# Pi-Star-Lab/RESCO

Hardware: AMD Instinct MI355X
Metric: env-steps/sec (higher is better)
Workload: dtype f32; 1 GPU; ingolstadt21 x 4096 lock-step envs per GPU (BASELINE config 3), fixed demand from the map's rou.xml, on-device seeded random policy, Krauss sigma 0.5 + speedFactor dev 0.1; tls_expiry=1, map=ingolstadt21, envs_per_gpu=4096, pipes=2, ticks_per_env_step=10, block_threads=512, lds_bytes_per_env=40896, parallelism=env-batch split x1, no collective on the data path

## Files before the change

resco_amd/csrc/resco_sim.hip:

```cpp
#include <hip/hip_runtime.h>
#include <hip/hip_fp16.h>
#include <stdint.h>
#include <stdio.h>
#include <stdlib.h>
#include <string.h>
#include <mutex>
#include <new>
#include <string>
#include <vector>

#include "resco_sim.h"

#define RS_DEV __device__ __forceinline__
#define RS_HD __host__ __device__
#define RS_MEM __device__ __forceinline__
#define RS_G(p) (p)
#define RS_CARVE __host__ __device__ __forceinline__
__device__ __forceinline__ void rs_atomic_min(int32_t *p, int32_t v) { atomicMin(p, v); }
__device__ __forceinline__ void rs_atomic_min(uint32_t *p, uint32_t v) { atomicMin(p, v); }
__device__ __forceinline__ void rs_atomic_max(int32_t *p, int32_t v) { atomicMax(p, v); }
__device__ __forceinline__ void rs_atomic_add(int32_t *p, int32_t v) { atomicAdd(p, v); }
__device__ __forceinline__ int32_t rs_atomic_fetch_add(int32_t *p, int32_t v) { return atomicAdd(p, v); }
__device__ __forceinline__ int32_t rs_wave_ticket(int32_t *p) {
    const unsigned long long m = __ballot(1);
    const int below = (int)__builtin_amdgcn_mbcnt_hi((uint32_t)(m >> 32), __builtin_amdgcn_mbcnt_lo((uint32_t)m, 0u));
    int32_t base = 0;
    if (below == 0) base = atomicAdd(p, (int32_t)__popcll(m));
    return __builtin_amdgcn_readlane(base, __ffsll((long long)m) - 1) + below;
}
__device__ __forceinline__ void rs_wave_add(int32_t *p, int32_t v) {
    for (int m = 32; m > 0; m >>= 1) v += __shfl_xor(v, m);
    if ((threadIdx.x & 63) == 0 && v) atomicAdd(p, v);
}
__device__ __forceinline__ void rs_wave_max(int32_t *p, int32_t v) {
    for (int m = 32; m > 0; m >>= 1) { const int32_t o = __shfl_xor(v, m); v = o > v ? o : v; }
    if ((threadIdx.x & 63) == 0) atomicMax(p, v);
}
__device__ __forceinline__ void rs_atomic_or(uint32_t *p, uint32_t v) { atomicOr(p, v); }
__device__ __forceinline__ uint32_t rs_atomic_fetch_or(uint32_t *p, uint32_t v) { return atomicOr(p, v); }
__device__ __forceinline__ int rs_atomic_inc(int32_t *p) { return atomicAdd(p, 1); }
__device__ __forceinline__ void rs_atomic_and(uint32_t *p, uint32_t v) { atomicAnd(p, v); }
__device__ __forceinline__ uint32_t rs_atomic_cas(uint32_t *p, uint32_t cmp, uint32_t v) { return atomicCAS(p, cmp, v); }
__device__ __forceinline__ int rs_ffsll(unsigned long long x) { return __ffsll(x); }
__device__ __forceinline__ int rs_clzll(unsigned long long x) { return __clzll((long long)x); }
__device__ __forceinline__ int rs_ffs(uint32_t x) { return __ffs((int)x); }
__device__ __forceinline__ int rs_popc(uint32_t x) { return __popc(x); }
__device__ __forceinline__ float rs_int_as_float(int x) { return __int_as_float(x); }
__device__ __forceinline__ int rs_float_as_int(float x) { return __float_as_int(x); }
__device__ __forceinline__ uint16_t rs_f2h(float x) { return __half_as_ushort(__float2half(x)); }

#ifndef RS_IEEE_DIV
__device__ __forceinline__ float rs_div_unscaled(float a, float b) {
    const float r0 = __builtin_amdgcn_rcpf(b);
    const float r1 = __builtin_fmaf(__builtin_fmaf(-b, r0, 1.0f), r0, r0);
    const float q0 = a * r1;
    const float q1 = __builtin_fmaf(__builtin_fmaf(-b, q0, a), r1, q0);
    return __builtin_fmaf(__builtin_fmaf(-b, q1, a), r1, q1);
}
#define RS_DIV(a, b) rs_div_unscaled((a), (b))
#endif
#define RS_OPAQUE_S(x) asm volatile("" : "+s"(x));
#ifndef RS_NARROW_NODE
#define RS_KEEP4(a, b, c, d) asm volatile("" : "+v"(a), "+v"(b), "+v"(c), "+v"(d));
#endif
extern __shared__ __attribute__((aligned(16))) char rs_smem[];
#define RS_SMEM rs_smem

#ifdef RS_STUDY_SECTIONS
__device__ unsigned long long *g_sec_prof;
#define RS_SEC_BEGIN unsigned long long sec_t = wall_clock64();
#define RS_SEC(id) { const unsigned long long sec_1 = wall_clock64(); if (g_sec_prof && (threadIdx.x & 63) == 0 && (blockIdx.x & 15) == 0) atomicAdd(&g_sec_prof[id], (sec_1 - sec_t) + (1ull << 40)); sec_t = wall_clock64(); }
#endif
#ifdef RS_DEVICE_ASSERT
#define RS_ASSERT(c) if (!(c)) rs_atomic_add(&L.sc[SC_STATS + ST_INVARIANT], 1);
#endif
#include "resco_host.h"
#include "resco_policy.h"
#include "resco_frap.h"

struct StepArgs { KTab T; State G; Out O; Lds L; };
typedef const __attribute__((address_space(4))) StepArgs *StepArgsPtr;

template <bool PROF> struct DevExec {
    int B;
    int wave;
    unsigned long long *prof;
    unsigned long long t0;
    template <class F> __device__ __forceinline__ void phase(int id, F f) {
        int w = wave;
        uint32_t ones = ~0u;
        asm volatile("" : "+s"(w), "+s"(ones));
        int tid = (w << 6) | (int)__builtin_amdgcn_mbcnt_hi(ones, __builtin_amdgcn_mbcnt_lo(ones, 0u));
        asm volatile("" : "+v"(tid));
        f(tid);
        __syncthreads();
        if (PROF && prof) {
            const unsigned long long t1 = wall_clock64();
            if (tid == 0) atomicAdd(&prof[id], t1 - t0);
            t0 = t1;
        }
    }
    __device__ __forceinline__ int wave_of(int) const { return wave; }
    __device__ __forceinline__ int next_chunk(int32_t *ctr, int, int, int) const {
        int c = 0;
        if (__builtin_amdgcn_mbcnt_hi(~0u, __builtin_amdgcn_mbcnt_lo(~0u, 0u)) == 0) c = atomicAdd(ctr, 1);
        return __builtin_amdgcn_readfirstlane(c);
    }
    __device__ __forceinline__ unsigned long long role_begin() const { return (PROF && prof) ? wall_clock64() : 0ull; }
    __device__ __forceinline__ void role_end(int id, unsigned long long start) const {
#ifdef RS_STUDY_SECTIONS
        return;
#endif
        if (PROF && prof && (threadIdx.x & 63) == 0 && (blockIdx.x & 15) == 0) atomicAdd(&prof[id], (wall_clock64() - start) + (1ull << 40));
    }
};
template <int CAP, bool PROF> __device__ __forceinline__ void rs_step_kernel_body(StepArgsPtr Ac, const KParams &P, const int32_t *__restrict__ actions) {
    if ((int)blockIdx.x >= P.n_envs) return;
    const StepArgs *A = (const StepArgs *)Ac;
#ifdef RS_STUDY_SECTIONS
    if (threadIdx.x == 0) g_sec_prof = P.prof;
#endif
    DevExec<PROF> ex{(int)blockDim.x, __builtin_amdgcn_readfirstlane((int)threadIdx.x >> 6), PROF ? P.prof : nullptr, (PROF && P.prof) ? wall_clock64() : 0ull};
    rs_step_body<CAP>(ex, A->L, A->T, A->G, A->O, P, actions, (int)blockIdx.x);
}
template <int CAP>
__global__ void __launch_bounds__(1024, 8)
rs_step_kernel_v64(StepArgsPtr Ac, KParams P, const int32_t *__restrict__ actions) { rs_step_kernel_body<CAP, false>(Ac, P, actions); }
template <int CAP>
__global__ void __launch_bounds__(768, 6)
rs_step_kernel_v80(StepArgsPtr Ac, KParams P, const int32_t *__restrict__ actions) { rs_step_kernel_body<CAP, false>(Ac, P, actions); }
template <int CAP>
__global__ void __launch_bounds__(512, 4)
rs_step_kernel_v128(StepArgsPtr Ac, KParams P, const int32_t *__restrict__ actions) { rs_step_kernel_body<CAP, false>(Ac, P, actions); }
__global__ void __launch_bounds__(768, 6)
rs_step_kernel_prof(StepArgsPtr Ac, KParams P, const int32_t *__restrict__ actions) { rs_step_kernel_body<0, true>(Ac, P, actions); }

__global__ void rs_reset_kernel(KTab T, State G, KParams P) { rs_reset_env(T, G, P, (int)blockIdx.x, (int)threadIdx.x, blockDim.x); }
__global__ void rs_reinit_kernel(KTab T, State G, KParams P) { rs_reinit_env(T, G, P, (int)blockIdx.x, (int)threadIdx.x, blockDim.x); }
__global__ void rs_act_random_kernel(KTab T, KParams P, uint32_t step_key, int32_t *actions) {
    const int i = blockIdx.x * blockDim.x + threadIdx.x;
    if (i < P.n_envs * T.n_signals) actions[i] = rs_random_action(T, P, step_key, i);
}
__global__ void rs_act_maxwave_kernel(KTab T, KParams P, const int32_t *pairs, int n_pairs, const int32_t *valid, const int32_t *order,
                                      int use_pressure, const int32_t *mplight, const int32_t *wave, int32_t *actions) {
    const int i = blockIdx.x * blockDim.x + threadIdx.x;
    if (i < P.n_envs * T.n_signals) actions[i] = rs_maxwave_action(T, pairs, n_pairs, valid, order, use_pressure, mplight, wave, i);
}

// ... 679 lines not shown
```

resco_amd/csrc/resco_step.h:

```cpp
#pragma once
#include "resco_tables.h"

struct State {
    char *base;
    size_t nc;
    int32_t *trip_log;
    int32_t *env;
    int32_t *tls;
    long long *stats;
    uint16_t *dep_next;
    uint32_t *mail;
    RS_HD float *pos() const { return (float *)base; }
    RS_HD float *speed() const { return RS_G((float *)(base + 4 * nc)); }
    RS_HD float *accel() const { return RS_G((float *)(base + 8 * nc)); }
    RS_HD float *tloss() const { return RS_G((float *)(base + 12 * nc)); }
    RS_HD float *sf() const { return RS_G((float *)(base + 16 * nc)); }
    RS_HD uint32_t *coop(int par) const { return RS_G((uint32_t *)(base + (par ? 43 : 20) * nc)); }
    RS_HD uint32_t *cooplead(int par) const { return RS_G((uint32_t *)(base + (par ? 47 : 24) * nc)); }
    RS_HD uint16_t *lane() const { return RS_G((uint16_t *)(base + 28 * nc)); }
    RS_HD uint16_t *trip() const { return RS_G((uint16_t *)(base + 30 * nc)); }
    RS_HD uint16_t *cursor() const { return RS_G((uint16_t *)(base + 32 * nc)); }
    RS_HD uint16_t *swait() const { return RS_G((uint16_t *)(base + 34 * nc)); }
    RS_HD uint16_t *rwait() const { return RS_G((uint16_t *)(base + 36 * nc)); }
    RS_HD uint16_t *depart() const { return RS_G((uint16_t *)(base + 38 * nc)); }
// ... 101 lines not shown
    uint16_t sfq;
};
#define FL_H 1
#define FL_MH 2
#define FL_LC 4
#define FL_MH1 8
RS_DEV int fl_mh(int t) { return (t & 1) ? FL_MH1 : FL_MH; }
#define LCT_LEFT 16
#define LCT_RIGHT 32
#define LCT_SWAP_LEFT 64
#define LCT_SWAP_RIGHT 128
struct __attribute__((aligned(8))) Aux {
    uint16_t lane, rq, nlink;
    uint16_t swait;
};
template <class Tp> struct LPtr {
    uint32_t off;
    RS_MEM Tp &operator[](int i) const { return ((Tp *)(RS_SMEM + off))[i]; }
    RS_MEM operator Tp *() const { return (Tp *)(RS_SMEM + off); }
};
struct Lds {
    LPtr<Node> node;
    LPtr<Aux> aux;
    LPtr<float> vnx, vtp;
    LPtr<uint16_t> grid;
    uint32_t gstride;
    LPtr<int32_t> arr;
    LPtr<uint16_t> dep, dep_t;
    LPtr<uint32_t> alive, alive0, insm;
    LPtr<uint32_t> mailw;
    LPtr<int32_t> agg_q, agg_a, agg_w, agg_m, agg_n;
    LPtr<uint32_t> agg_s;
    LPtr<int32_t> sig_arr, sig_dep;
    LPtr<int32_t> phase, left, nextp;
    LPtr<uint8_t> tstate;
    LPtr<int32_t> sc;
    LPtr<uint16_t> ls_h, ls_lc, ls_mh;
    uint32_t lcap;
    float cell_inv;
};
#define SC_T 0
#define SC_NINS 1
#define SC_HW 2
#define SC_NACT 3
#define SC_HWNEW 4
#define SC_ROOM 5
#define SC_HWOUT 6
#define SC_NH 7
#define SC_NLC 8
#define SC_NMH 9
#define SC_CHUNK_P 11
#define SC_CHUNK_M 12
#define SC_STATS 13
#ifndef RS_LIST_CHUNK
#define RS_LIST_CHUNK 64
#endif
#ifndef RS_H_CHUNK
#define RS_H_CHUNK RS_LIST_CHUNK
#endif

RS_CARVE size_t align16(size_t x) { return (x + 15) & ~(size_t)15; }
RS_CARVE int lds_list_cap(int C) {
#ifdef RS_LIST_CAP
    (void)C;
    return RS_LIST_CAP;
#else
    return ((C / 4 + 63) / 64) * 64;
#endif
}
RS_CARVE size_t lds_carve(Lds *L, int C, int n_cells, int n_arr, int n_dep, int n_obs, int S, int n_vt, int tls_maxl) {
    size_t o = 0;
#define CARVE(field, bytes) { if (L) L->field.off = (uint32_t)o; o += align16(bytes); }
    CARVE(node, (size_t)C * 16) CARVE(aux, (size_t)C * 8) CARVE(vnx, (size_t)C * 4)
    CARVE(sc, (size_t)(SC_STATS + ST_N) * 4)
    CARVE(alive, (size_t)((C + 31) / 32) * 4) CARVE(alive0, (size_t)((C + 31) / 32) * 4)
    {
        const int cap = lds_list_cap(C);
        if (L) L->lcap = (uint32_t)cap;
        CARVE(ls_h, (size_t)cap * 2) CARVE(ls_lc, (size_t)cap * 2) CARVE(ls_mh, (size_t)cap * 2)
    }
    const uint32_t grid_off = (uint32_t)o;
    const size_t grid_bytes = align16((size_t)((n_cells + 8 + 7) & ~7) * 2);
    if (L) L->gstride = (uint32_t)((n_cells + 8 + 7) & ~7);
    CARVE(grid, (size_t)((n_cells + 8 + 7) & ~7) * 2)
    CARVE(insm, (size_t)((n_dep + 31) / 32) * 4)
    CARVE(mailw, (size_t)((C + 31) / 32) * 4)
    CARVE(vtp, (size_t)n_vt * VT_COLS * 4)
    CARVE(phase, (size_t)S * 4) CARVE(left, (size_t)S * 4) CARVE(nextp, (size_t)S * 4)
    CARVE(sig_arr, (size_t)S * 4) CARVE(sig_dep, (size_t)S * 4)
    CARVE(tstate, (size_t)S * tls_maxl)
    CARVE(arr, (size_t)n_arr * 4) CARVE(dep, (size_t)n_dep * 2) CARVE(dep_t, (size_t)n_dep * 2)
    {
        const size_t ab = align16((size_t)n_obs * 4);
        uint32_t p = grid_off;
        if (6 * ab > grid_bytes) {
            p = (uint32_t)(align16((size_t)C * 16) + align16((size_t)C * 8));
            if (6 * ab > align16((size_t)C * 4)) { p = (uint32_t)o; o += 6 * ab; }
        }
        if (L) {
            L->agg_q.off = p; L->agg_a.off = p + (uint32_t)ab; L->agg_w.off = p + (uint32_t)(2 * ab);
            L->agg_m.off = p + (uint32_t)(3 * ab); L->agg_s.off = p + (uint32_t)(4 * ab); L->agg_n.off = p + (uint32_t)(5 * ab);
        }
    }
#undef CARVE
    return o;
}

template <class Tp, uint32_t OFF> struct CPtr {
    RS_MEM Tp &operator[](int i) const { return ((Tp *)(RS_SMEM + OFF))[i]; }
    RS_MEM operator Tp *() const { return (Tp *)(RS_SMEM + OFF); }
};
template <int C> struct LdsFix {
    static constexpr uint32_t a16(uint32_t x) { return (x + 15u) & ~15u; }
#ifdef RS_LIST_CAP
    static constexpr uint32_t kcap = RS_LIST_CAP;
#else
    static constexpr uint32_t kcap = ((C / 4 + 63) / 64) * 64;
#endif
    static constexpr uint32_t o_node = 0, o_aux = o_node + a16(C * 16), o_vnx = o_aux + a16(C * 8), o_sc = o_vnx + a16(C * 4),
                              o_alive = o_sc + a16((SC_STATS + ST_N) * 4), o_alive0 = o_alive + a16(((C + 31) / 32) * 4),
                              o_ls_h = o_alive0 + a16(((C + 31) / 32) * 4), o_ls_lc = o_ls_h + a16(kcap * 2), o_ls_mh = o_ls_lc + a16(kcap * 2),
                              o_grid = o_ls_mh + a16(kcap * 2);
    CPtr<Node, o_node> node;
    CPtr<Aux, o_aux> aux;
    CPtr<float, o_vnx> vnx;
    CPtr<int32_t, o_sc> sc;
    CPtr<uint32_t, o_alive> alive;
    CPtr<uint32_t, o_alive0> alive0;
    CPtr<uint16_t, o_ls_h> ls_h;
    CPtr<uint16_t, o_ls_lc> ls_lc;
    CPtr<uint16_t, o_ls_mh> ls_mh;
    CPtr<uint16_t, o_grid> grid;
    static constexpr uint32_t lcap = kcap;
    const LPtr<float> &vtp;
    const uint32_t &gstride;
    const LPtr<int32_t> &arr;
    const LPtr<uint16_t> &dep, &dep_t;
    const LPtr<uint32_t> &insm, &mailw;
    const LPtr<int32_t> &agg_q, &agg_a, &agg_w, &agg_m, &agg_n;
    const LPtr<uint32_t> &agg_s;
    const LPtr<int32_t> &sig_arr, &sig_dep, &phase, &left, &nextp;
    const LPtr<uint8_t> &tstate;
    const float &cell_inv;
    RS_MEM explicit LdsFix(const Lds &T)
        : vtp(T.vtp), gstride(T.gstride), arr(T.arr), dep(T.dep), dep_t(T.dep_t), insm(T.insm), mailw(T.mailw), agg_q(T.agg_q), agg_a(T.agg_a), agg_w(T.agg_w),
          agg_m(T.agg_m), agg_n(T.agg_n), agg_s(T.agg_s), sig_arr(T.sig_arr), sig_dep(T.sig_dep), phase(T.phase), left(T.left), nextp(T.nextp),
          tstate(T.tstate), cell_inv(T.cell_inv) {}
    static RS_HD bool matches(const Lds &T) {
        return T.node.off == o_node && T.aux.off == o_aux && T.vnx.off == o_vnx && T.sc.off == o_sc && T.alive.off == o_alive && T.alive0.off == o_alive0 &&
               T.ls_h.off == o_ls_h && T.ls_lc.off == o_ls_lc && T.ls_mh.off == o_ls_mh && T.grid.off == o_grid && T.lcap == kcap;
    }
};
RS_CARVE bool lds_fix_matches(const Lds &T, int C) {
    switch (C) {
        case 128: return LdsFix<128>::matches(T);
        case 256: return LdsFix<256>::matches(T);
        case 512: return LdsFix<512>::matches(T);
        case 768: return LdsFix<768>::matches(T);
        case 896: return LdsFix<896>::matches(T);
        case 1024: return LdsFix<1024>::matches(T);
        default: return true;
    }
}

RS_CARVE float pick_cell_len(const rs_scenario *sc, int n_arr, int n_dep, int tls_maxl) {
    const float choices[] = CELL_CHOICES;
    const int n = (int)(sizeof(choices) / sizeof(choices[0]));
    const size_t limits[2] = {RS_LDS_4WG_LIMIT, RS_LDS_3WG_LIMIT};
    for (int k = 0; k < 2; ++k)
        for (int i = 0; i < n; ++i)
            if (PackedTables::cell_len_ok(sc, choices[i]) &&
                lds_carve(nullptr, sc->capacity, PackedTables::count_cells(sc, choices[i]), n_arr, n_dep, sc->n_obs, sc->n_signals, sc->n_vtypes, tls_maxl) <= limits[k])
                return choices[i];
    for (int i = 0; i < n; ++i) if (PackedTables::cell_len_ok(sc, choices[i])) return choices[i];
    return choices[0];
}

#ifdef RS_EMU_DEBUG
#define RS_CHAIN_GUARD if (++rs_dbg_chain > 50000000L) { printf("endless chain walk\n"); fflush(stdout); abort(); }
#else
#define RS_CHAIN_GUARD
#endif
#ifndef RS_ASSERT
#define RS_ASSERT(c)
#endif
#ifndef RS_SEC
#define RS_SEC_BEGIN
#define RS_SEC(id) {}
#endif
template <class LT> RS_DEV int lane_cells(const LT &L, const LaneRec &LR) { return (int)(LR.len * L.cell_inv) + 1; }
template <class LT> RS_DEV int cell_of(const LT &L, float pos, int ncell) { const int c = (int)(pos * L.cell_inv); return c < ncell ? c : ncell - 1; }

struct Grid { uint16_t *c; uint32_t tag; };
RS_DEV unsigned long long grid_tag4(const Grid &g) { return g.tag ? 0x8000800080008000ull : 0ull; }
RS_DEV int cell_head(const Grid &g, int c) {
    const uint32_t v = g.c[c];
    return ((v ^ g.tag) & CELL_TAG) ? (int)NIL : (int)(v & NIL);
}
RS_DEV uint16_t grid_push(const Grid &g, int c, int s, bool mover) {
    uint32_t *w = (uint32_t *)g.c + (c >> 1);
    const int sh = (c & 1) * 16;
    const uint32_t flag = (mover ? CELL_MOVER : 0u) | g.tag;
    uint32_t old = *w, assumed, cell;
    do {
        assumed = old;
        cell = (assumed >> sh) & 0xFFFFu;
        if ((cell ^ g.tag) & CELL_TAG) cell = NIL;
        const uint32_t keep = cell & CELL_MOVER;
        uint32_t cnt = (cell >> CELL_CNT_SHIFT) & CELL_CNT_MAX;
        if (cnt < CELL_CNT_MAX) cnt += 1u;
        old = rs_atomic_cas(w, assumed, (assumed & ~(0xFFFFu << sh)) | (((uint32_t)s | (cnt << CELL_CNT_SHIFT) | keep | flag) << sh));
    } while (old != assumed);
    return (uint16_t)(cell & NIL);
}
RS_DEV unsigned long long quad_load(const Grid &g, int b) { return *(const unsigned long long *)(g.c + b) ^ grid_tag4(g); }
RS_DEV unsigned long long quad_occ(const Grid &g, int b) {
    const unsigned long long w = quad_load(g, b);
    const unsigned long long x = (w & 0x07FF07FF07FF07FFull) ^ 0x07FF07FF07FF07FFull;
    return (x + 0x07FF07FF07FF07FFull) & 0x0800080008000800ull & ~(w >> 4);
}
RS_DEV int cells_count(const Grid &g, int c0, int nc) {
    const int c1 = c0 + nc - 1;
    int n = 0;
    for (int b = c0 & ~3; b <= c1; b += 4) {
        const unsigned long long w = quad_load(g, b);
        unsigned long long m = (w >> CELL_CNT_SHIFT) & 0x0007000700070007ull;
        m &= ~(((w >> 15) & 0x0001000100010001ull) * 7ull);
        const int lo = c0 - b, hi = c1 - b;
        if (lo > 0) m &= ~0ull << (16 * lo);
        if (hi < 3) m &= ~0ull >> (16 * (3 - hi));
        n += (int)((m * 0x0001000100010001ull) >> 48);
    }
    return n;
}
RS_DEV int scan_up(const Grid &g, int c0, int c1) {
    for (int b = c0 & ~3; b <= c1; b += 4) {
        unsigned long long m = quad_occ(g, b);
        const int lo = c0 - b, hi = c1 - b;
        if (lo > 0) m &= ~0ull << (16 * lo);
        if (hi < 3) m &= ~0ull >> (16 * (3 - hi));
        if (m) return b + ((rs_ffsll(m) - 1) >> 4);
// ... 615 lines not shown
        const int b = overlapping(L, grid, (int)LR.cell0 + sdir * nc, nc, x, k, s, vt[VT_LENGTH]);
        if (b != NIL) {
            const Node nb = L.node[b];
            float rem_b;
            if (nb.speed <= RM_HALT_SPEED && (int)L.aux[b].swait >= RM_SWAP_WAIT &&
                strategic_dir(cont_row(T, L.aux[b].rq), kk + sdir, n, nb.pos, nb.speed, 0, rem_b, grid, (int)LR.cell0 + sdir * nc, nc, T.occ_unit) == -sdir && rem_b <= RM_URGENT_DIST &&
                overlapping(L, grid, LR.cell0, nc, nb.pos, nb.trip, b, L.vtp[nb.vt * VT_COLS + VT_LENGTH]) == s)
                code |= sdir > 0 ? LCT_SWAP_LEFT : LCT_SWAP_RIGHT;
        }
    }
        return code;
}

template <class LT> RS_DEV bool phase_insert_decide(const KTab &T, const LT &L, const Grid &grid, int t, int d) {
    if ((int)L.dep_t[d] > t) return false;
    const int k = L.dep[d];
    const DepInfo LR = T.cold.dep_info[d];
    const float *vt = L.vtp + T.trip_vtype()[k] * VT_COLS;
    const float mypos = vt[VT_LENGTH] < LR.len ? vt[VT_LENGTH] : LR.len;
    const int nc = (int)(LR.len * L.cell_inv) + 1;
    const int c1 = LR.cell0 + cell_of(L, mypos + vt[VT_MINGAP] + T.maxlen, nc);
    for (int c = scan_up(grid, LR.cell0, c1); c >= 0; c = (c < c1 ? scan_up(grid, c + 1, c1) : -1))
        for (int o = cell_head(grid, c); o != NIL;) { RS_CHAIN_GUARD
            const Node od = L.node[o];
            const float back = (od.pos + L.vnx[o]) - L.vtp[od.vt * VT_COLS + VT_LENGTH];
            if (back - mypos - vt[VT_MINGAP] < 0.0f) return false;
            o = od.nxt;
        }
    return true;
}

template <class LT> RS_DEV int nth_free_slot(const LT &L, int C, int r) {
#pragma unroll 1
    for (int w = 0; w < (C + 31) / 32; ++w) {
        uint32_t fr = ~L.alive0[w];
        if (w == (C - 1) / 32 && (C & 31)) fr &= (1u << (C & 31)) - 1u;
        const int c = rs_popc(fr);
        if (r >= c) { r -= c; continue; }
#pragma unroll 1
        for (int j = 0; j < r; ++j) fr &= fr - 1u;
        return w * 32 + rs_ffs(fr) - 1;
    }
    return -1;
}

template <class LT> RS_DEV void lc_decide_and_flag(const KTab &T, const LT &L, const Grid &grid, const State &G, size_t eo, int t, int s) {
    const Aux ax = L.aux[s];
    if (ax.lane == LANE_NONE) return;
    const int code = phase_lc_decide(T, L, grid, G, eo, t, s, ax, L.node[s]);
    if (code) flag_mover(L, s, t, code);
}
struct ExecInline {};

template <int CAP, class Exec, class LT>
RS_DEV void rs_step_body_on(Exec &ex, const LT &L, const KTab &T, const State &G, const Out &O, const KParams &P,
                            const int32_t *actions, int env) {
    const int B = ex.B;
    const int C = CAP ? CAP : T.capacity, S = T.n_signals, NO = T.n_obs;
    const int genv = P.env_base + env;
    const size_t eo = (size_t)env * C;
    const int n_ticks = P.n_ticks;

    uint16_t *const grid0 = L.grid;

    ex.phase(0, [&](int tid) {
        if (tid < SC_STATS + ST_N) L.sc[tid] = tid < 4 ? G.env[env * 4 + tid] : 0;
        for (int i = tid; i < T.n_vtypes * VT_COLS; i += B) L.vtp[i] = T.cold.vtype_params[i];
        for (int i = tid; i < (int)(L.gstride >> 1); i += B) ((uint32_t *)grid0)[i] = 0x07FF07FFu;
        for (int i = tid; i < T.n_arr; i += B) L.arr[i] = ARR_NONE;
        for (int i = tid; i < (C + 31) / 32; i += B) { L.alive[i] = 0u; L.mailw[i] = 0u; }
        for (int i = tid; i < (T.n_dep + 31) / 32; i += B) L.insm[i] = 0u;
        for (int i = tid; i < T.n_dep; i += B) {
            const int k = G.dep_next[(size_t)env * T.n_dep + i];
            L.dep[i] = (uint16_t)k;
            L.dep_t[i] = k == (int)TRIP_NONE ? (uint16_t)0xFFFF : (uint16_t)T.cold.trip_depart[k];
        }
        for (int i = tid; i < S; i += B) {
            const int ph = G.tls[(env * S + i) * TLS_W + 0];
            L.phase[i] = ph;
            L.left[i] = G.tls[(env * S + i) * TLS_W + 1];
            L.nextp[i] = G.tls[(env * S + i) * TLS_W + 2];
            L.sig_arr[i] = 0; L.sig_dep[i] = G.tls[(env * S + i) * TLS_W + 3];
            tls_refresh(T, L, P, i, ph);
        }
    });
    ex.phase(1, [&](int tid) {
        const int hw0 = L.sc[SC_HW];
        for (int s = tid; s < C; s += B) {
            uint16_t ln = LANE_NONE, tr = TRIP_NONE;
            if (s < hw0) { ln = G.lane()[eo + s]; tr = G.trip()[eo + s]; }
            Aux ax; ax.lane = ln; ax.rq = 0; ax.nlink = NLINK_NONE; ax.swait = 0;
            if (ln == LANE_NONE) { L.aux[s] = ax; L.node[s].trip = TRIP_NONE; continue; }
            const float sp = G.speed()[eo + s], x = G.pos()[eo + s];
            const int rq = (int)T.routes()[T.trip_route()[tr]].start + (int)G.cursor()[eo + s];
            const LaneRec LR0 = T.lanes()[ln];
            ax.rq = (uint16_t)rq;
            ax.nlink = cache_link(T, LR0, ln, rq, tr);
            ax.swait = G.swait()[eo + s];
            L.aux[s] = ax;
            Node nn; nn.pos = x; nn.speed = sp; nn.trip = tr; nn.vt = T.trip_vtype()[tr];
            nn.fl = 0; nn.sfq = (uint16_t)speed_factor_q(P, genv, tr, L.vtp + nn.vt * VT_COLS);
            if ((G.mail[(size_t)env * ((C + 31) / 32) + (s >> 5)] >> (s & 31)) & 1u) nn.sfq |= (uint16_t)SFQ_MAIL((L.sc[SC_T] + 1) & 1);
            nn.nxt = grid_push(Grid{grid0, 0u}, LR0.cell0 + cell_of(L, x, lane_cells(L, LR0)), s, sp > RM_HALT_SPEED);
            if (n_ticks > 0) nn.fl = (uint8_t)classify(T, L, s, L.vtp + nn.vt * VT_COLS, sp, x, LR0, ln, rq, T.notbest()[rq], tr, sf_of(nn.sfq), L.sc[SC_T]);
            L.node[s] = nn;
            rs_atomic_or(&L.alive[s >> 5], 1u << (s & 31));
        }
        for (int s = B - 1 - tid; s < S; s += B) {
            if (P.do_fsm && !P.fixed_program) {
                const int a = actions[env * S + s], cur = L.phase[s], Gn = T.cold.tls_ngreen[s];
                if (a < 0 || a >= T.cold.tls_nphase[s]) L.nextp[s] = cur;
                else {
                    L.nextp[s] = a;
                    if (cur != a && cur < Gn && a < Gn) {
                        const int y = T.cold.tls_yellow[T.cold.tls_yel_off[s] + cur * Gn + a];
                        if (y >= 0) set_phase(T, L, P, s, y);
                    }
                }
            }
            if (n_ticks > 0) tls_begin_of_tick(T, L, P, s, 0);
        }
    });
    if (n_ticks > 0) ex.phase(2, [&](int tid) {
        const int hw = L.sc[SC_HW];
        for (int s = tid; s < hw; s += B) {
            const Aux ax = L.aux[s];
            if (ax.lane == LANE_NONE) continue;
            const Node me = L.node[s];
            register_approach(T, L, ax.nlink, me.speed, me.pos, T.lanes()[ax.lane].len, me.vt);
        }
    });

    int cur = 0;
    for (int tick = 0; tick < n_ticks; ++tick) {
        const int t = L.sc[SC_T], hw = L.sc[cur ? SC_HWNEW : SC_HW];
        const Grid gold{grid0, cur ? CELL_TAG : 0u}, gnew{grid0, cur ? 0u : CELL_TAG};
        const bool more = tick + 1 < n_ticks;
        const int lcap = (int)L.lcap;
        const int nwv = B >> 6;
        ex.phase(4, [&](int tid) {
            const int wv = ex.wave_of(tid), ln = tid & 63;
            const int nh = L.sc[SC_NH], nlc = L.sc[SC_NLC];
            const unsigned long long r0 = ex.role_begin();
            int role = 0;
            if (nh > lcap || nlc > lcap) {
                for (int pass = 0; pass < 2; ++pass)
                    for (int w = tid; w < hw; w += B) {
                        if (pass && !(L.node[w].fl & FL_LC)) continue;
                        if (pass) lc_decide_and_flag(T, L, gold, G, eo, t, w);
                        else phase_plan<true>(T, L, gold, G, eo, P, genv, t, w);
                    }
            } else {
                const int hch = (nh + RS_H_CHUNK - 1) / RS_H_CHUNK, lch = (nlc + RS_LIST_CHUNK - 1) / RS_LIST_CHUNK;
                const int total = hch + lch + ((hw + 63) >> 6);
                for (int it = 0;; ++it) {
                    const int c = ex.next_chunk(&L.sc[SC_CHUNK_P], wv, it, nwv);
                    if (c >= total) break;
                    if (c < hch) {
                        role = 1;
                        const int w = c * RS_H_CHUNK + ln;
                        if (ln < RS_H_CHUNK && w < nh) phase_plan<true>(T, L, gold, G, eo, P, genv, t, L.ls_h[w]);
                    } else if (c < hch + lch) {
                        role = 2;
                        const int w = (c - hch) * RS_LIST_CHUNK + ln;
                        if (ln < RS_LIST_CHUNK && w < nlc) lc_decide_and_flag(T, L, gold, G, eo, t, L.ls_lc[w]);
                    } else {
                        const int w = (c - hch - lch) * 64 + ln;
                        if (w < hw && !(L.node[w].fl & FL_H)) phase_plan<false>(T, L, gold, G, eo, P, genv, t, w);
                    }
                }
            }
            ex.role_end(role == 1 ? 7 : (role == 2 ? 8 : 9), r0);
            for (int i = tid; i < (T.n_dep + 31) / 32; i += B) L.insm[i] = 0u;
        });
        ex.phase(5, [&](int tid) {
            for (int i = tid; i < T.n_arr; i += B) L.arr[i] = ARR_NONE;
            for (int i = tid; i < (C + 31) / 32; i += B) L.alive0[i] = L.alive[i];
            int Bs = B;
            RS_OPAQUE_S(Bs)
            for (int i = tid; i < (int)(L.gstride >> 2); i += Bs) {
                unsigned long long *q = (unsigned long long *)grid0 + i;
                const unsigned long long w = *q;
                const unsigned long long st = ((w ^ grid_tag4(gold)) >> 15) & 0x0001000100010001ull;
                if (st) { const unsigned long long m = st * 0xFFFFull; *q = (w & ~m) | ((0x07FF07FF07FF07FFull | grid_tag4(gold)) & m); }
            }
            for (int d = B - 1 - tid; d < T.n_dep; d += B)
                if (phase_insert_decide(T, L, gold, t, d)) rs_atomic_or(&L.insm[d >> 5], 1u << (d & 31));
            if (more)
                for (int sg = B - 1 - tid; sg < S; sg += B) tls_begin_of_tick(T, L, P, sg, tick + 1);
            if (tid == 0) {
                L.sc[SC_T] = t + 1; L.sc[SC_STATS + ST_TICKS] += 1;
                L.sc[cur ? SC_HW : SC_HWNEW] = 0;
                L.sc[SC_ROOM] = C - L.sc[SC_NACT];
                L.sc[SC_NH] = 0; L.sc[SC_NLC] = 0;
                L.sc[SC_NMH + ((t + 1) & 1)] = 0;
                L.sc[SC_CHUNK_P] = 0; L.sc[SC_CHUNK_M] = 0;
            }
        });
        ex.phase(6, [&](int tid) {
            int active = 0, halted = 0, top = 0;
            const int wv = ex.wave_of(tid), ln = tid & 63;
            const int nmh = L.sc[SC_NMH + (t & 1)];
            int ich = 0;
            for (int i = 0; i < (T.n_dep + 31) / 32; ++i) if (L.insm[i]) ich = 1;
            const bool all = nmh > lcap;
            const int mch = all ? 0 : (nmh + RS_LIST_CHUNK - 1) / RS_LIST_CHUNK;
            const int total = mch + ich + ((hw + 63) >> 6);
            const unsigned long long r0 = ex.role_begin();
            bool list = false;
            for (int it = 0;; ++it) {
                const int c = ex.next_chunk(&L.sc[SC_CHUNK_M], wv, it, nwv);
                if (c >= total) break;
                if (c < mch) {
                    list = true;
                    const int w = c * RS_LIST_CHUNK + ln;
                    if (ln < RS_LIST_CHUNK && w < nmh) phase_move<true>(T, L, gnew, G, P, env, eo, t, !more, more, L.ls_mh[w], active, halted, top);
                } else if (c < mch + ich) {
                    for (int d = 63 - ln; d < T.n_dep; d += 64) {
                        if (!(L.insm[d >> 5] & (1u << (d & 31)))) continue;
                        int rank = rs_popc(L.insm[d >> 5] & ((1u << (d & 31)) - 1u));
                        for (int w = 0; w < (d >> 5); ++w) rank += rs_popc(L.insm[w]);
                        if (rank >= L.sc[SC_ROOM]) { rs_atomic_add(&L.sc[SC_STATS + ST_CAP_BLOCKED], 1); continue; }
                        const int s = nth_free_slot(L, C, rank);
                        if (s < 0) continue;
                        const int k = L.dep[d];
                        const int v = T.trip_vtype()[k];
                        const float *vt = L.vtp + v * VT_COLS;
                        const RouteRec RR = T.routes()[T.trip_route()[k]];
                        const LaneRec LRd = T.lanes()[RR.depart_lane];
                        const int sfq = speed_factor_q(P, genv, k, vt);
                        const float sfn = sf_of(sfq);
                        Node nn; nn.pos = vt[VT_LENGTH] < RR.depart_len ? vt[VT_LENGTH] : RR.depart_len;
                        nn.speed = 0.0f; nn.trip = (uint16_t)k; nn.vt = (uint8_t)v; nn.fl = 0; nn.sfq = (uint16_t)sfq;
                        nn.nxt = grid_push(gnew, LRd.cell0 + cell_of(L, nn.pos, lane_cells(L, LRd)), s, false);
                        if (more) nn.fl = (uint8_t)classify(T, L, s, vt, 0.0f, nn.pos, LRd, RR.depart_lane, (int)RR.start, T.notbest()[RR.start], k, sfn, t + 1);
                        L.node[s] = nn;
                        Aux na; na.lane = RR.depart_lane; na.rq = (uint16_t)RR.start; na.swait = 0;
                        na.nlink = cache_link(T, LRd, RR.depart_lane, (int)RR.start, k);
                        L.aux[s] = na;
                        G.sf()[eo + s] = sfn; G.tloss()[eo + s] = 0.0f; G.cooplead(0)[eo + s] = COOP_NONE; G.cooplead(1)[eo + s] = COOP_NONE; G.coop(0)[eo + s] = COOP_NONE; G.coop(1)[eo + s] = COOP_NONE;
                        G.rwait()[eo + s] = 0; G.owner()[eo + s] = OWNER_NONE; G.depart()[eo + s] = (uint16_t)(t + 1); G.accel()[eo + s] = 0.0f; G.wtot()[eo + s] = 0;
                        {
                            const int k2 = T.cold.trip_next[k];
                            L.dep[d] = (uint16_t)k2;
                            L.dep_t[d] = k2 == (int)TRIP_NONE ? (uint16_t)0xFFFF : (uint16_t)T.cold.trip_depart[k2];
                        }
                        rs_atomic_or(&L.alive[s >> 5], 1u << (s & 31));
                        rs_atomic_add(&L.sc[SC_NACT], 1);
                        rs_atomic_add(&L.sc[SC_NINS], 1);
                        rs_atomic_add(&L.sc[SC_STATS + ST_INSERTED], 1);
                        rs_atomic_add(&L.sc[SC_STATS + ST_DEPDELAY], t - T.cold.trip_depart[k]);
// ... 16 lines not shown
        cur ^= 1;
    }
    const int hw_end = L.sc[cur ? SC_HWNEW : SC_HW];

    const bool obs = P.do_observe != 0;
    if (obs) ex.phase(11, [&](int tid) {
        for (int i = tid; i < NO; i += B) { L.agg_q[i] = 0; L.agg_a[i] = 0; L.agg_w[i] = 0; L.agg_m[i] = 0; L.agg_s[i] = 0; L.agg_n[i] = 0; }
    });
    ex.phase(12, [&](int tid) {
        const int hw0 = G.env[env * 4 + 2];
        const int top = hw_end > hw0 ? hw_end : hw0;
        int hi = 0;
        for (int s = tid; s < top; s += B) {
            const int lane = L.aux[s].lane;
            G.lane()[eo + s] = (uint16_t)lane; G.trip()[eo + s] = L.node[s].trip;
            if (lane == (int)LANE_NONE) continue;
            hi = s + 1;
            if (L.node[s].sfq & SFQ_MAIL((L.sc[SC_T] + 1) & 1)) rs_atomic_or(&L.mailw[s >> 5], 1u << (s & 31));
            const int rq = L.aux[s].rq;
            G.pos()[eo + s] = L.node[s].pos; G.speed()[eo + s] = L.node[s].speed; G.swait()[eo + s] = L.aux[s].swait;
            G.cursor()[eo + s] = (uint16_t)(rq - (int)T.routes()[T.trip_route()[L.node[s].trip]].start);
            if (!obs) continue;
            const int prev_owner = G.owner()[eo + s];
            const LaneRec LR = T.lanes()[lane];
            const int oi = T.cold.lane_obs[lane];
            bool detect = false;
            if (oi >= 0) {
                const float d = (LR.len - L.node[s].pos) + T.rsteps()[rq].tlsdist;
                detect = d <= P.max_distance;
            }
            if (!detect) {
                if (prev_owner != (int)OWNER_NONE) rs_atomic_add(&L.sig_dep[prev_owner], 1);
                G.owner()[eo + s] = OWNER_NONE; G.rwait()[eo + s] = 0;
                continue;
            }
            const int sig = T.cold.obs_sig[oi];
            int rw = G.rwait()[eo + s];
            if (prev_owner != sig) {
                rw = 0;
                rs_atomic_add(&L.sig_arr[sig], 1);
                rs_atomic_add(&L.agg_n[oi], 1);
                if (prev_owner != (int)OWNER_NONE) rs_atomic_add(&L.sig_dep[prev_owner], 1);
            }
            if (rw > 0) { rw += T.step_length; if (rw > 65535) rw = 65535; }
            else { const int sw = L.aux[s].swait; if (sw > 0) rw = sw; }
            G.rwait()[eo + s] = (uint16_t)rw;
            G.owner()[eo + s] = (uint8_t)sig;
            if (rw > 0) { rs_atomic_add(&L.agg_q[oi], 1); rs_atomic_add(&L.agg_w[oi], rw); rs_atomic_max(&L.agg_m[oi], rw); }
            else rs_atomic_add(&L.agg_a[oi], 1);
            rs_atomic_add((int32_t *)&L.agg_s[oi], (int32_t)(uint32_t)(L.node[s].speed * 65536.0f + 0.5f));
        }
        if (hi) rs_atomic_max(&L.sc[SC_HWOUT], hi);
    });
    ex.phase(13, [&](int tid) {
        const uint32_t om = obs ? P.out_mask : 0u;
        if (om & (OUT_LANE_AGG | OUT_DRQ_NORM)) for (int i = tid; i < NO * 5; i += B) {
            const int oi = i / 5, c = i - oi * 5;
            const int sg = T.cold.obs_sig[oi];
            const float sp = (float)L.agg_s[oi] * (1.0f / 65536.0f);
            float raw, nrm;
            if (c == 0) { raw = (float)L.agg_q[oi]; nrm = (oi - T.cold.sig_obs_start[sg]) == L.phase[sg] ? 1.0f : 0.0f; }
            else if (c == 1) { raw = (float)L.agg_a[oi]; nrm = raw / 28.0f; }
            else if (c == 2) { raw = (float)L.agg_w[oi]; nrm = raw / 28.0f; }
            else if (c == 3) { raw = (float)L.agg_m[oi]; nrm = (float)L.agg_q[oi] / 28.0f; }
            else { raw = sp; nrm = sp / 20.0f / 28.0f; }
            if (om & OUT_LANE_AGG) O.lane_agg()[(size_t)env * NO * 5 + i] = raw;
            if (om & OUT_DRQ_NORM) O.drq_norm()[(size_t)env * NO * 5 + i] = nrm;
        }
        if (om & OUT_LANE_ARR) for (int i = tid; i < NO; i += B) O.lane_arr()[(size_t)env * NO + i] = L.agg_n[i];
        if (om & OUT_DRQ_F16) for (int i = tid; i < S * T.lmax * 5; i += B) {
            const int sg = i / (T.lmax * 5), r = i - sg * T.lmax * 5;
            const int l = r / 5, c = r - l * 5;
            const int o0 = T.cold.sig_obs_start[sg];
            float nrm = 0.0f;
            if (l < T.cold.sig_obs_start[sg + 1] - o0) {
                const int oi = o0 + l;
                if (c == 0) nrm = l == L.phase[sg] ? 1.0f : 0.0f;
                else if (c == 1) nrm = (float)L.agg_a[oi] / 28.0f;
                else if (c == 2) nrm = (float)L.agg_w[oi] / 28.0f;
                else if (c == 3) nrm = (float)L.agg_q[oi] / 28.0f;
                else nrm = (float)L.agg_s[oi] * (1.0f / 65536.0f) / 20.0f / 28.0f;
            }
            O.drq_f16()[(size_t)env * S * T.lmax * 5 + i] = rs_f2h(nrm);
        }
        if (om & (OUT_MPLIGHT | OUT_WAVE | OUT_MPLIGHT_FULL)) for (int i = tid; i < S * 12; i += B) {
            const int sg = i / 12, m = i - sg * 12;
            int q = 0, wv = 0, tw = 0, ap = 0;
            float last_speed = 0.0f;
            for (int j = T.cold.mv_in_start[i]; j < T.cold.mv_in_start[i + 1]; ++j) {
                const int oi = T.cold.mv_in_idx[j];
                q += L.agg_q[oi]; wv += L.agg_q[oi] + L.agg_a[oi]; tw += L.agg_w[oi]; ap += L.agg_a[oi];
                last_speed = (float)L.agg_s[oi] * (1.0f / 65536.0f);
            }
            for (int j = T.cold.mv_out_start[i]; j < T.cold.mv_out_start[i + 1]; ++j) q -= L.agg_q[T.cold.mv_out_idx[j]];
            const size_t so = (size_t)env * S + sg;
            if (om & OUT_MPLIGHT) O.mplight()[so * 13 + 1 + m] = q;
            if (om & OUT_WAVE) O.wave()[so * 12 + m] = wv;
            if (om & OUT_MPLIGHT_FULL) {
                float *mf = O.mplight_full() + so * 49 + 1 + m * 4;
                mf[0] = (float)q; mf[1] = (float)tw / 28.0f; mf[2] = last_speed; mf[3] = (float)ap / 28.0f;
            }
        }
        for (int sg = tid; sg < S; sg += B) {
            const int ph = L.phase[sg];
            if (obs) {
                const int o0 = T.cold.sig_obs_start[sg], o1 = T.cold.sig_obs_start[sg + 1];
                int tw = 0, tq = 0, mq = 0;
                for (int oi = o0; oi < o1; ++oi) { tw += L.agg_w[oi]; const int qq = L.agg_q[oi]; tq += qq; if (qq > mq) mq = qq; }
                const size_t so = (size_t)env * S + sg;
                O.phase()[so] = ph; O.queue_sum()[so] = tq; O.queue_max()[so] = mq;
                O.wait()[so] = -(float)tw;
                const float wn = -(float)tw / 224.0f;
                O.wait_norm()[so] = wn < -4.0f ? -4.0f : (wn > 4.0f ? 4.0f : wn);
                int pr = tq;
                for (int i = T.cold.pr_out_start[sg]; i < T.cold.pr_out_start[sg + 1]; ++i) pr -= L.agg_q[T.cold.pr_out_idx[i]];
                O.pressure()[so] = -pr;
                if (om & OUT_MPLIGHT) O.mplight()[so * 13] = ph;
                if (om & OUT_MPLIGHT_FULL) O.mplight_full()[so * 49] = (float)ph;
                O.arrivals()[so] = L.sig_arr[sg]; O.departures()[so] = L.sig_dep[sg];
            }
            G.tls[(env * S + sg) * TLS_W + 0] = ph;
            G.tls[(env * S + sg) * TLS_W + 1] = L.left[sg];
            G.tls[(env * S + sg) * TLS_W + 2] = L.nextp[sg];
            G.tls[(env * S + sg) * TLS_W + 3] = obs ? 0 : L.sig_dep[sg];
        }
        for (int i = tid; i < T.n_dep; i += B) G.dep_next[(size_t)env * T.n_dep + i] = L.dep[i];
        for (int i = tid; i < (C + 31) / 32; i += B) G.mail[(size_t)env * ((C + 31) / 32) + i] = L.mailw[i];
    });
    ex.phase(14, [&](int tid) {
        if (tid == 0) {
            G.env[env * 4 + 0] = L.sc[SC_T]; G.env[env * 4 + 1] = L.sc[SC_NINS]; G.env[env * 4 + 3] = L.sc[SC_NACT];
            G.env[env * 4 + 2] = L.sc[SC_HWOUT];
        }
        if (tid < ST_N) {
            long long *st = G.stats + (size_t)env * ST_N;
            if (tid == ST_ACTIVE) st[tid] = L.sc[SC_NACT];
            else if (tid == ST_PENDING) {
                const int t = L.sc[SC_T];
                const int hz = t - 1 <= T.horizon ? t - 1 : T.horizon;
                st[tid] = (t >= 1 ? T.cold.trips_cum[hz] : 0) - L.sc[SC_NINS];
            } else st[tid] += L.sc[SC_STATS + tid];
        }
    });
}

template <int CAP, class Exec>
RS_DEV void rs_step_body(Exec &ex, const Lds &L, const KTab &T, const State &G, const Out &O, const KParams &P,
                         const int32_t *actions, int env) {
    if constexpr (CAP != 0) {
        const LdsFix<CAP> Lf(L);
        rs_step_body_on<CAP>(ex, Lf, T, G, O, P, actions, env);
    } else rs_step_body_on<CAP>(ex, L, T, G, O, P, actions, env);
}
```

Baseline: 3.886 million env-steps/s.

## Fold tick tail into plan phase via last-wave arrival and drop barriers

Removes the per-tick phase-5 barrier. The last wave to finish phase 4, detected with an LDS arrival counter, runs the arrival reset, the compacted insert check and the TLS begin-of-tick work alone. The grid tag sweep and alive0 copy move into phase 4's dynamic chunk queue. Phase 2 is merged into phase 1 (action handling into phase 0, approach registration into node load), and phases 13 and 14 are fused with no trailing barrier. This saves several workgroup barriers per tick, but serializes the tail onto one wave and depends on fence correctness.

```diff
diff --git a/resco_amd/csrc/resco_sim.hip b/resco_amd/csrc/resco_sim.hip
--- a/resco_amd/csrc/resco_sim.hip
+++ b/resco_amd/csrc/resco_sim.hip
@@ -63,13 +63,34 @@
 #ifndef RS_NARROW_NODE
 #define RS_KEEP4(a, b, c, d) asm volatile("" : "+v"(a), "+v"(b), "+v"(c), "+v"(d));
 #endif
+#define RS_TAIL_WIDTH 64
+__device__ __forceinline__ bool rs_wave_arrive(int32_t *ctr, int n) {
+    __builtin_amdgcn_fence(__ATOMIC_RELEASE, "workgroup");
+    int c = 0;
+    if (__builtin_amdgcn_mbcnt_hi(~0u, __builtin_amdgcn_mbcnt_lo(~0u, 0u)) == 0) c = atomicAdd(ctr, 1);
+    const bool last = __builtin_amdgcn_readfirstlane(c) == n - 1;
+    if (last) __builtin_amdgcn_fence(__ATOMIC_ACQUIRE, "workgroup");
+    return last;
+}
+#define RS_WAVE_ARRIVE(c, n, B) rs_wave_arrive((c), (n))
+#define RS_TEAM_SYNC __builtin_amdgcn_fence(__ATOMIC_ACQ_REL, "wavefront"); __builtin_amdgcn_wave_barrier();
+#define RS_LAST_PHASE(ex, id, f) (ex).template phase<false>((id), (f))
 extern __shared__ __attribute__((aligned(16))) char rs_smem[];
 #define RS_SMEM rs_smem
 
 #ifdef RS_STUDY_SECTIONS
 __device__ unsigned long long *g_sec_prof;
-#define RS_SEC_BEGIN unsigned long long sec_t = wall_clock64();
-#define RS_SEC(id) { const unsigned long long sec_1 = wall_clock64(); if (g_sec_prof && (threadIdx.x & 63) == 0 && (blockIdx.x & 15) == 0) atomicAdd(&g_sec_prof[id], (sec_1 - sec_t) + (1ull << 40)); sec_t = wall_clock64(); }
+#define RS_SEC_T0_ unsigned long long sec_t = wall_clock64();
+#define RS_SEC_ADD_(id) { const unsigned long long sec_1 = wall_clock64(); if (g_sec_prof && (threadIdx.x & 63) == 0 && (blockIdx.x & 15) == 0) atomicAdd(&g_sec_prof[id], (sec_1 - sec_t) + (1ull << 40)); sec_t = wall_clock64(); }
+#ifdef RS_STUDY_C
+#define RS_SEC_BEGIN
+#define RS_SEC(id) {}
+#define RS_SECC_BEGIN RS_SEC_T0_
+#define RS_SECC(id) RS_SEC_ADD_(id)
+#else
+#define RS_SEC_BEGIN RS_SEC_T0_
+#define RS_SEC(id) RS_SEC_ADD_(id)
+#endif
 #endif
 #ifdef RS_DEVICE_ASSERT
 #define RS_ASSERT(c) if (!(c)) rs_atomic_add(&L.sc[SC_STATS + ST_INVARIANT], 1);
@@ -86,14 +107,14 @@
     int wave;
     unsigned long long *prof;
     unsigned long long t0;
-    template <class F> __device__ __forceinline__ void phase(int id, F f) {
+    template <bool BARRIER = true, class F> __device__ __forceinline__ void phase(int id, F f) {
         int w = wave;
         uint32_t ones = ~0u;
         asm volatile("" : "+s"(w), "+s"(ones));
         int tid = (w << 6) | (int)__builtin_amdgcn_mbcnt_hi(ones, __builtin_amdgcn_mbcnt_lo(ones, 0u));
         asm volatile("" : "+v"(tid));
         f(tid);
-        __syncthreads();
+        if (BARRIER) __syncthreads();
         if (PROF && prof) {
             const unsigned long long t1 = wall_clock64();
             if (tid == 0) atomicAdd(&prof[id], t1 - t0);
diff --git a/resco_amd/csrc/resco_step.h b/resco_amd/csrc/resco_step.h
--- a/resco_amd/csrc/resco_step.h
+++ b/resco_amd/csrc/resco_step.h
@@ -177,6 +177,9 @@
 #define SC_CHUNK_P 11
 #define SC_CHUNK_M 12
 #define SC_STATS 13
+#define SC_ARRIVE (SC_STATS + ST_N)
+#define SC_NDUE (SC_STATS + ST_N + 1)
+#define SC_END (SC_STATS + ST_N + 2)
 #ifndef RS_LIST_CHUNK
 #define RS_LIST_CHUNK 64
 #endif
@@ -197,7 +200,7 @@
     size_t o = 0;
 #define CARVE(field, bytes) { if (L) L->field.off = (uint32_t)o; o += align16(bytes); }
     CARVE(node, (size_t)C * 16) CARVE(aux, (size_t)C * 8) CARVE(vnx, (size_t)C * 4)
-    CARVE(sc, (size_t)(SC_STATS + ST_N) * 4)
+    CARVE(sc, (size_t)SC_END * 4)
     CARVE(alive, (size_t)((C + 31) / 32) * 4) CARVE(alive0, (size_t)((C + 31) / 32) * 4)
     {
         const int cap = lds_list_cap(C);
@@ -243,7 +246,7 @@
     static constexpr uint32_t kcap = ((C / 4 + 63) / 64) * 64;
 #endif
     static constexpr uint32_t o_node = 0, o_aux = o_node + a16(C * 16), o_vnx = o_aux + a16(C * 8), o_sc = o_vnx + a16(C * 4),
-                              o_alive = o_sc + a16((SC_STATS + ST_N) * 4), o_alive0 = o_alive + a16(((C + 31) / 32) * 4),
+                              o_alive = o_sc + a16(SC_END * 4), o_alive0 = o_alive + a16(((C + 31) / 32) * 4),
                               o_ls_h = o_alive0 + a16(((C + 31) / 32) * 4), o_ls_lc = o_ls_h + a16(kcap * 2), o_ls_mh = o_ls_lc + a16(kcap * 2),
                               o_grid = o_ls_mh + a16(kcap * 2);
     CPtr<Node, o_node> node;
@@ -312,6 +315,10 @@
 #ifndef RS_SEC
 #define RS_SEC_BEGIN
 #define RS_SEC(id) {}
+#endif
+#ifndef RS_SECC
+#define RS_SECC_BEGIN
+#define RS_SECC(id) {}
 #endif
 template <class LT> RS_DEV int lane_cells(const LT &L, const LaneRec &LR) { return (int)(LR.len * L.cell_inv) + 1; }
 template <class LT> RS_DEV int cell_of(const LT &L, float pos, int ncell) { const int c = (int)(pos * L.cell_inv); return c < ncell ? c : ncell - 1; }
@@ -1033,6 +1040,48 @@
 }
 struct ExecInline {};
 
+#ifndef RS_C_TAIL
+#define RS_C_TAIL 1
+#endif
+#ifndef RS_TAIL_WIDTH
+#define RS_TAIL_WIDTH 1
+#endif
+#ifndef RS_WAVE_ARRIVE
+#define RS_WAVE_ARRIVE(c, n, B) (rs_atomic_fetch_add((c), 1) == (B) - 1)
+#endif
+#ifndef RS_TEAM_SYNC
+#define RS_TEAM_SYNC
+#endif
+#ifndef RS_LAST_PHASE
+#define RS_LAST_PHASE(ex, id, f) (ex).phase((id), (f))
+#endif
+#define RS_SWEEP_Q 4
+RS_DEV void grid_sweep_quad(uint16_t *grid0, const Grid &gold, int i) {
+    unsigned long long *q = (unsigned long long *)grid0 + i;
+    const unsigned long long w = *q;
+    const unsigned long long st = ((w ^ grid_tag4(gold)) >> 15) & 0x0001000100010001ull;
+    if (st) { const unsigned long long m = st * 0xFFFFull; *q = (w & ~m) | ((0x07FF07FF07FF07FFull | grid_tag4(gold)) & m); }
+}
+template <class LT> RS_DEV void insert_check(const KTab &T, const LT &L, const Grid &gold, int t, int ln) {
+    const int W = RS_TAIL_WIDTH, lcap = (int)L.lcap;
+    for (int i = ln; i < (T.n_dep + 31) / 32; i += W) L.insm[i] = 0u;
+    for (int d = ln; d < T.n_dep; d += W)
+        if ((int)L.dep_t[d] <= t) {
+            const int i = rs_wave_ticket(&L.sc[SC_NDUE]);
+            if (i < lcap) L.ls_h[i] = (uint16_t)d;
+        }
+    RS_TEAM_SYNC
+    const int nd = L.sc[SC_NDUE];
+    const bool ovf = nd > lcap;
+    const int n = ovf ? T.n_dep : nd;
+    for (int j = ln; j < n; j += W) {
+        const int d = ovf ? j : (int)L.ls_h[j];
+        if (phase_insert_decide(T, L, gold, t, d)) rs_atomic_or(&L.insm[d >> 5], 1u << (d & 31));
+    }
+    RS_TEAM_SYNC
+    if (ln == 0) L.sc[SC_NDUE] = 0;
+}
+
 template <int CAP, class Exec, class LT>
 RS_DEV void rs_step_body_on(Exec &ex, const LT &L, const KTab &T, const State &G, const Out &O, const KParams &P,
                             const int32_t *actions, int env) {
@@ -1045,7 +1094,7 @@
     uint16_t *const grid0 = L.grid;
 
     ex.phase(0, [&](int tid) {
-        if (tid < SC_STATS + ST_N) L.sc[tid] = tid < 4 ? G.env[env * 4 + tid] : 0;
+        if (tid < SC_END) L.sc[tid] = tid < 4 ? G.env[env * 4 + tid] : 0;
         for (int i = tid; i < T.n_vtypes * VT_COLS; i += B) L.vtp[i] = T.cold.vtype_params[i];
         for (int i = tid; i < (int)(L.gstride >> 1); i += B) ((uint32_t *)grid0)[i] = 0x07FF07FFu;
         for (int i = tid; i < T.n_arr; i += B) L.arr[i] = ARR_NONE;
@@ -1063,6 +1112,18 @@
             L.nextp[i] = G.tls[(env * S + i) * TLS_W + 2];
             L.sig_arr[i] = 0; L.sig_dep[i] = G.tls[(env * S + i) * TLS_W + 3];
             tls_refresh(T, L, P, i, ph);
+            if (P.do_fsm && !P.fixed_program) {
+                const int a = actions[env * S + i], cur = ph, Gn = T.cold.tls_ngreen[i];
+                if (a < 0 || a >= T.cold.tls_nphase[i]) L.nextp[i] = cur;
+                else {
+                    L.nextp[i] = a;
+                    if (cur != a && cur < Gn && a < Gn) {
+                        const int y = T.cold.tls_yellow[T.cold.tls_yel_off[i] + cur * Gn + a];
+                        if (y >= 0) set_phase(T, L, P, i, y);
+                    }
+                }
+            }
+            if (n_ticks > 0) tls_begin_of_tick(T, L, P, i, 0);
         }
     });
     ex.phase(1, [&](int tid) {
@@ -1086,29 +1147,7 @@
             if (n_ticks > 0) nn.fl = (uint8_t)classify(T, L, s, L.vtp + nn.vt * VT_COLS, sp, x, LR0, ln, rq, T.notbest()[rq], tr, sf_of(nn.sfq), L.sc[SC_T]);
             L.node[s] = nn;
             rs_atomic_or(&L.alive[s >> 5], 1u << (s & 31));
-        }
-        for (int s = B - 1 - tid; s < S; s += B) {
-            if (P.do_fsm && !P.fixed_program) {
-                const int a = actions[env * S + s], cur = L.phase[s], Gn = T.cold.tls_ngreen[s];
-                if (a < 0 || a >= T.cold.tls_nphase[s]) L.nextp[s] = cur;
-                else {
-                    L.nextp[s] = a;
-                    if (cur != a && cur < Gn && a < Gn) {
-                        const int y = T.cold.tls_yellow[T.cold.tls_yel_off[s] + cur * Gn + a];
-                        if (y >= 0) set_phase(T, L, P, s, y);
-                    }
-                }
-            }
-            if (n_ticks > 0) tls_begin_of_tick(T, L, P, s, 0);
-        }
-    });
-    if (n_ticks > 0) ex.phase(2, [&](int tid) {
-        const int hw = L.sc[SC_HW];
-        for (int s = tid; s < hw; s += B) {
-            const Aux ax = L.aux[s];
-            if (ax.lane == LANE_NONE) continue;
-            const Node me = L.node[s];
-            register_approach(T, L, ax.nlink, me.speed, me.pos, T.lanes()[ax.lane].len, me.vt);
+            if (n_ticks > 0) register_approach(T, L, ax.nlink, sp, x, LR0.len, nn.vt);
         }
     });
 
@@ -1119,11 +1158,21 @@
         const bool more = tick + 1 < n_ticks;
         const int lcap = (int)L.lcap;
         const int nwv = B >> 6;
+        auto c_scalars = [&]() {
+            L.sc[SC_T] = t + 1; L.sc[SC_STATS + ST_TICKS] += 1;
+            L.sc[cur ? SC_HW : SC_HWNEW] = 0;
+            L.sc[SC_ROOM] = C - L.sc[SC_NACT];
+            L.sc[SC_NH] = 0; L.sc[SC_NLC] = 0;
+            L.sc[SC_NMH + ((t + 1) & 1)] = 0;
+            L.sc[SC_CHUNK_P] = 0; L.sc[SC_CHUNK_M] = 0;
+        };
         ex.phase(4, [&](int tid) {
             const int wv = ex.wave_of(tid), ln = tid & 63;
             const int nh = L.sc[SC_NH], nlc = L.sc[SC_NLC];
             const unsigned long long r0 = ex.role_begin();
             int role = 0;
+            for (int i = tid; i < (C + 31) / 32; i += B) L.alive0[i] = L.alive[i];
+            const int nq = (int)(L.gstride >> 2);
             if (nh > lcap || nlc > lcap) {
                 for (int pass = 0; pass < 2; ++pass)
                     for (int w = tid; w < hw; w += B) {
@@ -1131,12 +1180,16 @@
                         if (pass) lc_decide_and_flag(T, L, gold, G, eo, t, w);
                         else phase_plan<true>(T, L, gold, G, eo, P, genv, t, w);
                     }
+                int Bs = B;
+                RS_OPAQUE_S(Bs)
+                for (int i = tid; i < nq; i += Bs) grid_sweep_quad(grid0, gold, i);
             } else {
                 const int hch = (nh + RS_H_CHUNK - 1) / RS_H_CHUNK, lch = (nlc + RS_LIST_CHUNK - 1) / RS_LIST_CHUNK;
                 const int total = hch + lch + ((hw + 63) >> 6);
+                const int sch = (nq + 64 * RS_SWEEP_Q - 1) / (64 * RS_SWEEP_Q);
                 for (int it = 0;; ++it) {
                     const int c = ex.next_chunk(&L.sc[SC_CHUNK_P], wv, it, nwv);
-                    if (c >= total) break;
+                    if (c >= total + sch) break;
                     if (c < hch) {
                         role = 1;
                         const int w = c * RS_H_CHUNK + ln;
@@ -1145,39 +1198,47 @@
                         role = 2;
                         const int w = (c - hch) * RS_LIST_CHUNK + ln;
                         if (ln < RS_LIST_CHUNK && w < nlc) lc_decide_and_flag(T, L, gold, G, eo, t, L.ls_lc[w]);
-                    } else {
+                    } else if (c < total) {
                         const int w = (c - hch - lch) * 64 + ln;
                         if (w < hw && !(L.node[w].fl & FL_H)) phase_plan<false>(T, L, gold, G, eo, P, genv, t, w);
+                    } else {
+                        const int i0 = (c - total) * (64 * RS_SWEEP_Q) + ln;
+#pragma unroll
+                        for (int j = 0; j < RS_SWEEP_Q; ++j) if (i0 + 64 * j < nq) grid_sweep_quad(grid0, gold, i0 + 64 * j);
                     }
                 }
             }
             ex.role_end(role == 1 ? 7 : (role == 2 ? 8 : 9), r0);
-            for (int i = tid; i < (T.n_dep + 31) / 32; i += B) L.insm[i] = 0u;
+#if RS_C_TAIL
+            if (RS_WAVE_ARRIVE(&L.sc[SC_ARRIVE], nwv, B)) {
+                RS_SECC_BEGIN
+                const int W = RS_TAIL_WIDTH, tl = tid & (RS_TAIL_WIDTH - 1);
+                for (int i = tl; i < T.n_arr; i += W) L.arr[i] = ARR_NONE;
+                RS_SECC(7)
+                insert_check(T, L, gold, t, tl);
+                RS_SECC(8)
+                if (more)
+                    for (int sg = tl; sg < S; sg += W) tls_begin_of_tick(T, L, P, sg, tick + 1);
+                RS_SECC(9)
+                if (tl == 0) { c_scalars(); L.sc[SC_ARRIVE] = 0; }
+                RS_SECC(10)
+            }
+#endif
         });
+#if !RS_C_TAIL
         ex.phase(5, [&](int tid) {
+            RS_SECC_BEGIN
             for (int i = tid; i < T.n_arr; i += B) L.arr[i] = ARR_NONE;
-            for (int i = tid; i < (C + 31) / 32; i += B) L.alive0[i] = L.alive[i];
-            int Bs = B;
-            RS_OPAQUE_S(Bs)
-            for (int i = tid; i < (int)(L.gstride >> 2); i += Bs) {
-                unsigned long long *q = (unsigned long long *)grid0 + i;
-                const unsigned long long w = *q;
-                const unsigned long long st = ((w ^ grid_tag4(gold)) >> 15) & 0x0001000100010001ull;
-                if (st) { const unsigned long long m = st * 0xFFFFull; *q = (w & ~m) | ((0x07FF07FF07FF07FFull | grid_tag4(gold)) & m); }
-            }
-            for (int d = B - 1 - tid; d < T.n_dep; d += B)
-                if (phase_insert_decide(T, L, gold, t, d)) rs_atomic_or(&L.insm[d >> 5], 1u << (d & 31));
+            RS_SECC(7)
+            if (tid >= B - RS_TAIL_WIDTH) insert_check(T, L, gold, t, tid & (RS_TAIL_WIDTH - 1));
+            RS_SECC(8)
             if (more)
-                for (int sg = B - 1 - tid; sg < S; sg += B) tls_begin_of_tick(T, L, P, sg, tick + 1);
-            if (tid == 0) {
-                L.sc[SC_T] = t + 1; L.sc[SC_STATS + ST_TICKS] += 1;
-                L.sc[cur ? SC_HW : SC_HWNEW] = 0;
-                L.sc[SC_ROOM] = C - L.sc[SC_NACT];
-                L.sc[SC_NH] = 0; L.sc[SC_NLC] = 0;
-                L.sc[SC_NMH + ((t + 1) & 1)] = 0;
-                L.sc[SC_CHUNK_P] = 0; L.sc[SC_CHUNK_M] = 0;
-            }
+                for (int sg = tid; sg < S; sg += B) tls_begin_of_tick(T, L, P, sg, tick + 1);
+            RS_SECC(9)
+            if (tid == 0) c_scalars();
+            RS_SECC(10)
         });
+#endif
         ex.phase(6, [&](int tid) {
             int active = 0, halted = 0, top = 0;
             const int wv = ex.wave_of(tid), ln = tid & 63;
@@ -1300,7 +1361,7 @@
         }
         if (hi) rs_atomic_max(&L.sc[SC_HWOUT], hi);
     });
-    ex.phase(13, [&](int tid) {
+    auto outputs = [&](int tid) {
         const uint32_t om = obs ? P.out_mask : 0u;
         if (om & (OUT_LANE_AGG | OUT_DRQ_NORM)) for (int i = tid; i < NO * 5; i += B) {
             const int oi = i / 5, c = i - oi * 5;
@@ -1374,8 +1435,6 @@
         }
         for (int i = tid; i < T.n_dep; i += B) G.dep_next[(size_t)env * T.n_dep + i] = L.dep[i];
         for (int i = tid; i < (C + 31) / 32; i += B) G.mail[(size_t)env * ((C + 31) / 32) + i] = L.mailw[i];
-    });
-    ex.phase(14, [&](int tid) {
         if (tid == 0) {
             G.env[env * 4 + 0] = L.sc[SC_T]; G.env[env * 4 + 1] = L.sc[SC_NINS]; G.env[env * 4 + 3] = L.sc[SC_NACT];
             G.env[env * 4 + 2] = L.sc[SC_HWOUT];
@@ -1389,7 +1448,8 @@
                 st[tid] = (t >= 1 ? T.cold.trips_cum[hz] : 0) - L.sc[SC_NINS];
             } else st[tid] += L.sc[SC_STATS + tid];
         }
-    });
+    };
+    RS_LAST_PHASE(ex, 13, outputs);
 }
 
 template <int CAP, class Exec>
```

Result: slower. 3.717 million env-steps/s (-4.4%).
